# VainF/Diff-Pruning

Hardware: AMD Instinct MI355X
Metric: importance-scored images/sec (UNet fwd+bwd+|w*dL/dw|) (higher is better)
Workload: dtype f32

## Files before the change

diff-pruning_amd/csrc/wgrad2d.hip:

```cpp
#include <cstdlib>
#include "dp_common.h"

#define DPG2_RSRC_FLAGS 0x00020000
#define DPG2_OOB 0x80000000u
typedef __attribute__((address_space(3))) void dpg2_lds_void;

__device__ __forceinline__ __amdgpu_buffer_rsrc_t dpg2_rsrc(const float* base, unsigned bytes) {
    return __builtin_amdgcn_make_buffer_rsrc((void*)base, 0, (int)bytes, DPG2_RSRC_FLAGS);
}

template <int LW, bool TAIL>
__device__ __forceinline__ void wgrad_wino2d_body(const dp_nt_gemm_params& p) {
    constexpr int W = 1 << LW, TC = W / 2, LTC = LW - 1;
    constexpr int PA = 68;
    constexpr int NXC = 16 + W / 2;
    constexpr int PB = 4 * NXC + 4;
    constexpr int A_SLOTS = 64 * 17, B_SLOTS = 32 * (NXC + 1);
    constexpr int NA = (A_SLOTS + 255) / 256, NB = (B_SLOTS + 255) / 256;
    constexpr int A_SZ = NA * 1024, B_SZ = NB * 1024;
    constexpr int STAGE = A_SZ + B_SZ;
    __shared__ __attribute__((aligned(16))) float smem[(2 * STAGE > 12288) ? 2 * STAGE : 12288];

    const int tid = threadIdx.x;
    const int lane = tid & 63;
    const int wave = __builtin_amdgcn_readfirstlane(tid >> 6);
    const int m0 = blockIdx.y * 64, n0 = blockIdx.x * 32;
    const int split = blockIdx.z;
    const dp_conv_geom& g = p.g;
    const int H = g.Ho, HW = H * W;
    const int lhw = 31 - __builtin_clz((unsigned)HW);
    const int C1 = p.X2 ? g.c_split : p.NCOLS;
    const bool src1 = n0 < C1;
    const float* Xs = src1 ? p.X1 : p.X2;
    const int ncs = src1 ? C1 : p.NCOLS - C1;
    const int cb = src1 ? n0 : n0 - C1;
    const long long xis = src1 ? g.x1_img_stride : g.x2_img_stride;
    const int T = p.P >> 6;
    const int tps = p.p_per_split >> 6;
    const int t0 = split * tps, t1 = min(t0 + tps, T);
    const int nIter = t1 - t0;

    const __amdgpu_buffer_rsrc_t rA = dpg2_rsrc(p.A, p.a_bytes);
    const __amdgpu_buffer_rsrc_t rB = dpg2_rsrc(Xs, src1 ? p.x1_bytes : p.x2_bytes);
    unsigned a_c[NA], b_c[NB];
    int b_dr[NB];
#pragma unroll
    for (int j = 0; j < NA; ++j) {
        const int q = 256 * j + tid;
        const int row = q / 17, s = q - 17 * row;
        a_c[j] = (q < A_SLOTS && s < 16 && m0 + row < p.M) ? (unsigned)(((m0 + row) * HW + 4 * s) * 4) : DPG2_OOB;
    }
#pragma unroll
    for (int j = 0; j < NB; ++j) {
        const int q = 256 * j + tid;
        const int row = q / (NXC + 1), s = q - (NXC + 1) * row;
        b_c[j] = (q < B_SLOTS && s < NXC && cb + row < ncs) ? (unsigned)(((cb + row) * HW + 4 * s) * 4) : DPG2_OOB;
        b_dr[j] = (4 * s) >> LW;
    }
    float* const ldsA = smem + 4 * (wave * 64);
    float* const ldsB = smem + A_SZ + 4 * (wave * 64);

    auto dma_tile = [&](int t, int buf) {
        const int pb = 64 * t;
        const int img = pb >> lhw, r = pb & (HW - 1);
        const int R0 = r >> LW;
        const unsigned a_s = (unsigned)((long long)img * p.a_img_stride + r) * 4u;
        const long long b_base = (long long)img * xis + r - W;
#pragma unroll
        for (int j = 0; j < NA; ++j) {
            unsigned oa = a_c[j] != DPG2_OOB ? a_c[j] + a_s : DPG2_OOB;
            asm volatile("" : "+v"(oa));
            __builtin_amdgcn_raw_ptr_buffer_load_lds(rA, (dpg2_lds_void*)(ldsA + buf * STAGE + 1024 * j), 16, (int)oa, 0, 0, 0);
        }
#pragma unroll
        for (int j = 0; j < NB; ++j) {
            const bool v = b_c[j] != DPG2_OOB && (unsigned)(R0 - 1 + b_dr[j]) < (unsigned)H;
            unsigned ob = v ? (unsigned)((long long)b_c[j] + b_base * 4) : DPG2_OOB;
            asm volatile("" : "+v"(ob));
            __builtin_amdgcn_raw_ptr_buffer_load_lds(rB, (dpg2_lds_void*)(ldsB + buf * STAGE + 1024 * j), 16, (int)ob, 0, 0, 0);
        }
    };

    f32x16 acc[4][2];
#pragma unroll
    for (int j = 0; j < 4; ++j)
#pragma unroll
        for (int t = 0; t < 2; ++t)
#pragma unroll
            for (int r = 0; r < 16; ++r) acc[j][t][r] = 0.f;

    const int li = lane & 31, lk = lane >> 5;
    const float* fragA = smem + li * PA + 2 * lk;
    const float* fragB = smem + A_SZ + li * PB + 2 * lk;
    const float s0 = wave == 3 ? 0.f : 1.f, s1 = wave == 0 ? 0.f : wave == 1 ? 1.f : -1.f;
    const int ra = wave == 0 ? 0 : wave == 2 ? 2 : 1;
    const int rb = wave == 0 ? 2 : wave == 1 ? 2 : wave == 2 ? 1 : 3;
    const float sgn = wave == 1 ? 1.f : -1.f;
    const bool lk0 = lk == 0, lk1 = lk == 1;

    if (nIter > 0) {
        dma_tile(t0, 0);
        asm volatile("s_waitcnt vmcnt(0)" ::: "memory");
        __syncthreads();
        if (TAIL && m0 + 32 >= p.M) {
#define G2_NT 1
#include "wgrad2d_kloop.inc"
#undef G2_NT
        } else {
#define G2_NT 2
#include "wgrad2d_kloop.inc"
#undef G2_NT
        }
    }

    float* hbuf = smem;
    const int o_cs = p.o_col_stride ? p.o_col_stride : p.ntaps;
    const long long o_ts = p.o_tap_stride ? p.o_tap_stride : 1;
    float* __restrict__ outb = p.out + (long long)split * p.o_bs;
    const int col = n0 + li;
    const bool col_ok = col < p.NCOLS && !(src1 && col >= C1);
#pragma unroll
    for (int t = 0; t < 2; ++t) {
        if (t) __syncthreads();
#pragma unroll
        for (int r = 0; r < 16; ++r) {
            const float hs = 0.5f * (acc[1][t][r] + acc[2][t][r]);
            hbuf[((wave * 3 + 0) * 16 + r) * 64 + lane] = acc[0][t][r] + hs;
            hbuf[((wave * 3 + 1) * 16 + r) * 64 + lane] = 0.5f * (acc[1][t][r] - acc[2][t][r]);
            hbuf[((wave * 3 + 2) * 16 + r) * 64 + lane] = hs + acc[3][t][r];
        }
        __syncthreads();
        if (!col_ok) continue;
#pragma unroll
        for (int q4 = 0; q4 < 4; ++q4) {
            const int r = 4 * wave + q4;
            const int m = m0 + 32 * t + (r & 3) + 8 * (r >> 2) + 4 * lk;
            float h[4][3];
#pragma unroll
            for (int i = 0; i < 4; ++i)
#pragma unroll
                for (int b = 0; b < 3; ++b) h[i][b] = hbuf[((i * 3 + b) * 16 + r) * 64 + lane];
            if (m >= p.M) continue;
#pragma unroll
            for (int b = 0; b < 3; ++b) {
                const float hs = 0.5f * (h[1][b] + h[2][b]);
                const float w3[3] = {h[0][b] + hs, 0.5f * (h[1][b] - h[2][b]), hs + h[3][b]};
#pragma unroll
                for (int a = 0; a < 3; ++a) {
                    float* o = outb + (long long)(3 * a + b) * o_ts + (long long)m * p.ldo + (long long)col * o_cs;
                    float v = p.alpha * w3[a];
                    if (p.accumulate) v += *o;
                    *o = v;
                }
            }
        }
    }
}

template <int LW>
__global__ __launch_bounds__(256, 2) void wgrad_wino2d_kernel(const dp_nt_gemm_params p) {
    wgrad_wino2d_body<LW, false>(p);
}
template <int LW>
__global__ __launch_bounds__(256, 2) void wgrad_wino2d_tail_kernel(const dp_nt_gemm_params p) {
    wgrad_wino2d_body<LW, true>(p);
}

static bool wgrad_wino2d_ok(const dp_nt_gemm_params& p) {
    const dp_conv_geom& g = p.g;
    if (p.batched || p.merge || p.col_bias || p.ntaps != 9 || g.kw != 3 || g.stride != 1 || g.sden != 1 || g.ups) return false;
    if (g.pad_t != 1 || g.pad_l != 1 || g.Ho != g.Hs || g.Wo != g.Ws || g.Hs != g.Hv || g.Ws != g.Wv) return false;
    const int W = g.Wo, HW = g.Ho * g.Wo;
    if ((W != 8 && W != 16 && W != 32) || (HW & (HW - 1)) || HW < 64 || (g.Ho & 1)) return false;
    if ((p.P % 64) || (p.p_per_split % 64) || p.p_per_split <= 0) return false;
    if ((unsigned long long)p.x1_bytes >= 0x80000000ull || (p.X2 && (unsigned long long)p.x2_bytes >= 0x80000000ull)) return false;
    if (p.X2 && (g.c_split % 32)) return false;
    return true;
}

extern "C" int dp_wgrad_wino2d_supported(const dp_nt_gemm_params* p) { return wgrad_wino2d_ok(*p) ? 1 : 0; }

extern "C" int dp_wgrad_wino2d(const dp_nt_gemm_params* pp, void* stream) {
    const dp_nt_gemm_params& p = *pp;
    if (p.M <= 0 || p.NCOLS <= 0) return 0;
    if (!wgrad_wino2d_ok(p) || p.splits <= 0 || (long long)p.splits * p.p_per_split < (long long)p.P) return (int)hipErrorInvalidValue;
    const int C1 = p.X2 ? p.g.c_split : p.NCOLS;
    dim3 grid((C1 + 31) / 32 + (p.X2 ? (p.NCOLS - C1 + 31) / 32 : 0), (p.M + 63) / 64, p.splits);
    hipStream_t st = (hipStream_t)stream;
    static const bool tail_off = [] { const char* e = getenv("DP_WINO2D_TAIL"); return e && atoi(e) == 0; }();
    const bool tail = !tail_off && (p.M & 63) >= 1 && (p.M & 63) <= 32;
    if (tail) {
        if (p.g.Wo == 32)      DP_LAUNCH((wgrad_wino2d_tail_kernel<5>), grid, dim3(256), 0, st, p);
        else if (p.g.Wo == 16) DP_LAUNCH((wgrad_wino2d_tail_kernel<4>), grid, dim3(256), 0, st, p);
        else                   DP_LAUNCH((wgrad_wino2d_tail_kernel<3>), grid, dim3(256), 0, st, p);
        return DP_LAUNCH_CHECK();
    }
    if (p.g.Wo == 32)      DP_LAUNCH((wgrad_wino2d_kernel<5>), grid, dim3(256), 0, st, p);
    else if (p.g.Wo == 16) DP_LAUNCH((wgrad_wino2d_kernel<4>), grid, dim3(256), 0, st, p);
    else                   DP_LAUNCH((wgrad_wino2d_kernel<3>), grid, dim3(256), 0, st, p);
    return DP_LAUNCH_CHECK();
}
```

Measured before the change: 5063.

## Use eight-wavefront workgroups for Winograd wgrad at W>=16 with XCD-aware block remap

For 16- and 32-wide feature maps, the Winograd weight-gradient kernel now launches 512-thread workgroups. Two groups of four waves each own one 32-row half of the M tile, so each wave keeps a single accumulator set instead of two, which relieves register pressure and adds waves for latency hiding. The A and B DMA loads are merged into one per-wave slot loop sized to the new thread count. The epilogue is split across the two wave groups. An XCD-aware remapping of block indices is also added, so that consecutive logical tiles land on the same XCD for L2 locality.

```diff
diff --git a/diff-pruning_amd/csrc/wgrad2d.hip b/diff-pruning_amd/csrc/wgrad2d.hip
--- a/diff-pruning_amd/csrc/wgrad2d.hip
+++ b/diff-pruning_amd/csrc/wgrad2d.hip
@@ -5,27 +5,60 @@
 #define DPG2_OOB 0x80000000u
 typedef __attribute__((address_space(3))) void dpg2_lds_void;
 
+constexpr int dpg2_waves(int LW) {
+#ifdef DPG2_WAVES
+    return (void)LW, DPG2_WAVES;
+#else
+    return LW >= 4 ? 8 : 4;
+#endif
+}
+constexpr bool dpg2_xcd(int NW) {
+#ifdef DPG2_XCD
+    return (void)NW, DPG2_XCD != 0;
+#else
+    return NW == 8;
+#endif
+}
+
 __device__ __forceinline__ __amdgpu_buffer_rsrc_t dpg2_rsrc(const float* base, unsigned bytes) {
     return __builtin_amdgcn_make_buffer_rsrc((void*)base, 0, (int)bytes, DPG2_RSRC_FLAGS);
 }
 
-template <int LW, bool TAIL>
+template <int LW, bool TAIL, int NW>
 __device__ __forceinline__ void wgrad_wino2d_body(const dp_nt_gemm_params& p) {
     constexpr int W = 1 << LW, TC = W / 2, LTC = LW - 1;
     constexpr int PA = 68;
     constexpr int NXC = 16 + W / 2;
     constexpr int PB = 4 * NXC + 4;
     constexpr int A_SLOTS = 64 * 17, B_SLOTS = 32 * (NXC + 1);
-    constexpr int NA = (A_SLOTS + 255) / 256, NB = (B_SLOTS + 255) / 256;
-    constexpr int A_SZ = NA * 1024, B_SZ = NB * 1024;
-    constexpr int STAGE = A_SZ + B_SZ;
+    static_assert((NW == 4 || NW == 8) && !(TAIL && NW == 8), "the tail form is a four-wavefront body");
+    constexpr int NT = 8 / NW;
+    constexpr int NAI = NW == 4 ? 4 * ((A_SLOTS + 255) / 256) : A_SLOTS / 64;
+    constexpr int NBI = NW == 4 ? 4 * ((B_SLOTS + 255) / 256) : (B_SLOTS + 63) / 64;
+    constexpr int NR = (NAI + NBI + NW - 1) / NW;
+    constexpr int A_SZ = NAI * 256;
+    constexpr int STAGE = NR * NW * 256;
+    static_assert(A_SLOTS % 64 == 0 && NR * NW * 64 >= NAI * 64 + B_SLOTS && 2 * STAGE * 4 <= 81920, "two workgroups per CU");
     __shared__ __attribute__((aligned(16))) float smem[(2 * STAGE > 12288) ? 2 * STAGE : 12288];
 
     const int tid = threadIdx.x;
     const int lane = tid & 63;
-    const int wave = __builtin_amdgcn_readfirstlane(tid >> 6);
-    const int m0 = blockIdx.y * 64, n0 = blockIdx.x * 32;
-    const int split = blockIdx.z;
+    const int wv = __builtin_amdgcn_readfirstlane(tid >> 6);
+    const int wave = wv & 3;
+    const int grp = wv >> 2;
+    int bx = blockIdx.x, by = blockIdx.y, split = blockIdx.z;
+    if (dpg2_xcd(NW)) {
+        const int gxy = gridDim.x * gridDim.y;
+        const int nwg = gxy * gridDim.z;
+        const int b = blockIdx.x + gridDim.x * (blockIdx.y + gridDim.y * blockIdx.z);
+        const int q8 = nwg >> 3, r8 = nwg & 7, xcd = b & 7, k8 = b >> 3;
+        const int v = (xcd < r8 ? xcd * (q8 + 1) : r8 * (q8 + 1) + (xcd - r8) * q8) + k8;
+        split = __builtin_amdgcn_readfirstlane(v / gxy);
+        const int rem = v - split * gxy;
+        by = __builtin_amdgcn_readfirstlane(rem / (int)gridDim.x);
+        bx = rem - by * (int)gridDim.x;
+    }
+    const int m0 = by * 64, n0 = bx * 32;
     const dp_conv_geom& g = p.g;
     const int H = g.Ho, HW = H * W;
     const int lhw = 31 - __builtin_clz((unsigned)HW);
@@ -42,55 +75,48 @@
 
     const __amdgpu_buffer_rsrc_t rA = dpg2_rsrc(p.A, p.a_bytes);
     const __amdgpu_buffer_rsrc_t rB = dpg2_rsrc(Xs, src1 ? p.x1_bytes : p.x2_bytes);
-    unsigned a_c[NA], b_c[NB];
-    int b_dr[NB];
-#pragma unroll
-    for (int j = 0; j < NA; ++j) {
-        const int q = 256 * j + tid;
+    unsigned ld_c[NR];
+    int ld_dr[NR];
+    bool ld_a[NR];
+#pragma unroll
+    for (int j = 0; j < NR; ++j) {
+        ld_a[j] = NW * (j + 1) <= NAI ? true : NW * j >= NAI ? false : NW * j + wv < NAI;
+        const int q = 64 * NW * j + tid;
         const int row = q / 17, s = q - 17 * row;
-        a_c[j] = (q < A_SLOTS && s < 16 && m0 + row < p.M) ? (unsigned)(((m0 + row) * HW + 4 * s) * 4) : DPG2_OOB;
-    }
-#pragma unroll
-    for (int j = 0; j < NB; ++j) {
-        const int q = 256 * j + tid;
-        const int row = q / (NXC + 1), s = q - (NXC + 1) * row;
-        b_c[j] = (q < B_SLOTS && s < NXC && cb + row < ncs) ? (unsigned)(((cb + row) * HW + 4 * s) * 4) : DPG2_OOB;
-        b_dr[j] = (4 * s) >> LW;
-    }
-    float* const ldsA = smem + 4 * (wave * 64);
-    float* const ldsB = smem + A_SZ + 4 * (wave * 64);
+        const unsigned ca = (q < A_SLOTS && s < 16 && m0 + row < p.M) ? (unsigned)(((m0 + row) * HW + 4 * s) * 4) : DPG2_OOB;
+        const int qb = q - 64 * NAI;
+        const int rowb = qb / (NXC + 1), sb = qb - (NXC + 1) * rowb;
+        const unsigned cx = (qb >= 0 && qb < B_SLOTS && sb < NXC && cb + rowb < ncs) ? (unsigned)(((cb + rowb) * HW + 4 * sb) * 4) : DPG2_OOB;
+        ld_c[j] = ld_a[j] ? ca : cx;
+        ld_dr[j] = ld_a[j] ? 1 : (4 * sb) >> LW;
+    }
+    float* const ldsW = smem + 4 * (wv * 64);
 
     auto dma_tile = [&](int t, int buf) {
         const int pb = 64 * t;
         const int img = pb >> lhw, r = pb & (HW - 1);
         const int R0 = r >> LW;
         const unsigned a_s = (unsigned)((long long)img * p.a_img_stride + r) * 4u;
-        const long long b_base = (long long)img * xis + r - W;
-#pragma unroll
-        for (int j = 0; j < NA; ++j) {
-            unsigned oa = a_c[j] != DPG2_OOB ? a_c[j] + a_s : DPG2_OOB;
-            asm volatile("" : "+v"(oa));
-            __builtin_amdgcn_raw_ptr_buffer_load_lds(rA, (dpg2_lds_void*)(ldsA + buf * STAGE + 1024 * j), 16, (int)oa, 0, 0, 0);
-        }
-#pragma unroll
-        for (int j = 0; j < NB; ++j) {
-            const bool v = b_c[j] != DPG2_OOB && (unsigned)(R0 - 1 + b_dr[j]) < (unsigned)H;
-            unsigned ob = v ? (unsigned)((long long)b_c[j] + b_base * 4) : DPG2_OOB;
-            asm volatile("" : "+v"(ob));
-            __builtin_amdgcn_raw_ptr_buffer_load_lds(rB, (dpg2_lds_void*)(ldsB + buf * STAGE + 1024 * j), 16, (int)ob, 0, 0, 0);
+        const unsigned b_s = (unsigned)(((long long)img * xis + r - W) * 4);
+#pragma unroll
+        for (int j = 0; j < NR; ++j) {
+            const bool v = ld_c[j] != DPG2_OOB && (ld_a[j] || (unsigned)(R0 - 1 + ld_dr[j]) < (unsigned)H);
+            unsigned o = v ? ld_c[j] + (ld_a[j] ? a_s : b_s) : DPG2_OOB;
+            asm volatile("" : "+v"(o));
+            __builtin_amdgcn_raw_ptr_buffer_load_lds(ld_a[j] ? rA : rB, (dpg2_lds_void*)(ldsW + buf * STAGE + 256 * NW * j), 16, (int)o, 0, 0, 0);
         }
     };
 
-    f32x16 acc[4][2];
+    f32x16 acc[4][NT];
 #pragma unroll
     for (int j = 0; j < 4; ++j)
 #pragma unroll
-        for (int t = 0; t < 2; ++t)
+        for (int t = 0; t < NT; ++t)
 #pragma unroll
             for (int r = 0; r < 16; ++r) acc[j][t][r] = 0.f;
 
     const int li = lane & 31, lk = lane >> 5;
-    const float* fragA = smem + li * PA + 2 * lk;
+    const float* fragA = smem + (NW == 8 ? 32 * grp * PA : 0) + li * PA + 2 * lk;
     const float* fragB = smem + A_SZ + li * PB + 2 * lk;
     const float s0 = wave == 3 ? 0.f : 1.f, s1 = wave == 0 ? 0.f : wave == 1 ? 1.f : -1.f;
     const int ra = wave == 0 ? 0 : wave == 2 ? 2 : 1;
@@ -102,7 +128,7 @@
         dma_tile(t0, 0);
         asm volatile("s_waitcnt vmcnt(0)" ::: "memory");
         __syncthreads();
-        if (TAIL && m0 + 32 >= p.M) {
+        if (NW == 8 || (TAIL && m0 + 32 >= p.M)) {
 #define G2_NT 1
 #include "wgrad2d_kloop.inc"
 #undef G2_NT
@@ -122,18 +148,21 @@
 #pragma unroll
     for (int t = 0; t < 2; ++t) {
         if (t) __syncthreads();
-#pragma unroll
-        for (int r = 0; r < 16; ++r) {
-            const float hs = 0.5f * (acc[1][t][r] + acc[2][t][r]);
-            hbuf[((wave * 3 + 0) * 16 + r) * 64 + lane] = acc[0][t][r] + hs;
-            hbuf[((wave * 3 + 1) * 16 + r) * 64 + lane] = 0.5f * (acc[1][t][r] - acc[2][t][r]);
-            hbuf[((wave * 3 + 2) * 16 + r) * 64 + lane] = hs + acc[3][t][r];
+        constexpr int ti = NW == 8 ? 0 : 1;
+        if (NW == 4 || grp == t) {
+#pragma unroll
+            for (int r = 0; r < 16; ++r) {
+                const float hs = 0.5f * (acc[1][t * ti][r] + acc[2][t * ti][r]);
+                hbuf[((wave * 3 + 0) * 16 + r) * 64 + lane] = acc[0][t * ti][r] + hs;
+                hbuf[((wave * 3 + 1) * 16 + r) * 64 + lane] = 0.5f * (acc[1][t * ti][r] - acc[2][t * ti][r]);
+                hbuf[((wave * 3 + 2) * 16 + r) * 64 + lane] = hs + acc[3][t * ti][r];
+            }
         }
         __syncthreads();
         if (!col_ok) continue;
 #pragma unroll
-        for (int q4 = 0; q4 < 4; ++q4) {
-            const int r = 4 * wave + q4;
+        for (int q4 = 0; q4 < 16 / NW; ++q4) {
+            const int r = 16 / NW * wv + q4;
             const int m = m0 + 32 * t + (r & 3) + 8 * (r >> 2) + 4 * lk;
             float h[4][3];
 #pragma unroll
@@ -158,12 +187,12 @@
 }
 
 template <int LW>
-__global__ __launch_bounds__(256, 2) void wgrad_wino2d_kernel(const dp_nt_gemm_params p) {
-    wgrad_wino2d_body<LW, false>(p);
+__global__ __launch_bounds__(64 * dpg2_waves(LW), 2) void wgrad_wino2d_kernel(const dp_nt_gemm_params p) {
+    wgrad_wino2d_body<LW, false, dpg2_waves(LW)>(p);
 }
 template <int LW>
 __global__ __launch_bounds__(256, 2) void wgrad_wino2d_tail_kernel(const dp_nt_gemm_params p) {
-    wgrad_wino2d_body<LW, true>(p);
+    wgrad_wino2d_body<LW, true, 4>(p);
 }
 
 static bool wgrad_wino2d_ok(const dp_nt_gemm_params& p) {
@@ -195,8 +224,8 @@
         else                   DP_LAUNCH((wgrad_wino2d_tail_kernel<3>), grid, dim3(256), 0, st, p);
         return DP_LAUNCH_CHECK();
     }
-    if (p.g.Wo == 32)      DP_LAUNCH((wgrad_wino2d_kernel<5>), grid, dim3(256), 0, st, p);
-    else if (p.g.Wo == 16) DP_LAUNCH((wgrad_wino2d_kernel<4>), grid, dim3(256), 0, st, p);
-    else                   DP_LAUNCH((wgrad_wino2d_kernel<3>), grid, dim3(256), 0, st, p);
+    if (p.g.Wo == 32)      DP_LAUNCH((wgrad_wino2d_kernel<5>), grid, dim3(64 * dpg2_waves(5)), 0, st, p);
+    else if (p.g.Wo == 16) DP_LAUNCH((wgrad_wino2d_kernel<4>), grid, dim3(64 * dpg2_waves(4)), 0, st, p);
+    else                   DP_LAUNCH((wgrad_wino2d_kernel<3>), grid, dim3(64 * dpg2_waves(3)), 0, st, p);
     return DP_LAUNCH_CHECK();
 }
```

Measured after the change: 5071 (median of 6 runs). Within noise of the previous version (+0.2%).
